# courtois-neuromod/phantom_vlb

Measured on AMD Instinct MI355X. Metric: clips/sec fine-tune VideoLLaMA2-7B+LoRA->2k-voxel head, 1/2/4/8 MI355X, higher is better.
Workload: dtype bf16; 1 GPU; configs[2]: VideoLLaMA2-7B + LoRA r=16 + 2k-voxel head, bf16; clips_per_gpu=3, global_batch=3, seq_len=2048, frames=12, num_target=2048, weights=random-init, comm=none

## Files before the change

### include/vlb.h

```cpp
#ifndef VLB_H
#define VLB_H

#include <stdint.h>

#ifdef __cplusplus
extern "C" {
#endif
#if defined(__GNUC__) || defined(__clang__)
#pragma GCC visibility push(default)
#endif

#define VLB_OK 0
#define VLB_ERR_INVALID (-1)
#define VLB_ERR_LAUNCH (-2)

#define VLB_ABI_VERSION 2

#define VLB_ACT_NONE 0
#define VLB_ACT_QUICK_GELU 1
#define VLB_ACT_GELU 2
#define VLB_ACT_SILU 3
#define VLB_ACT_SWIGLU_PAIR 4
#define VLB_ACT_SWIGLU_BWD 5

// ... 18 lines not shown
                              void* stream);

int vlb_gemm_bf16_masked_pair_ws(const void* A, int lda, const void* W, int ldw, void* C, int ldc, int M, int N, int K,
                                 const void* A2, int lda2, const void* W2, int ldw2, float drop_p, uint32_t seed,
                                 void* ws, int64_t ws_bytes, void* stream);

int vlb_gemm_masked_pair_swiglu_bwd(const void* dY, int lddy, const void* Wt, int ldw, const void* gu, int ldgu, void* dgu,
                                    int lddgu, int M, int ff, int K, const void* U, int ldu, const void* At, int ldat,
                                    float drop_p, uint32_t seed, void* ws, int64_t ws_bytes, void* stream);

int vlb_gemm_kernel_choice(int M, int N, int K, int K2);

int vlb_transpose_bf16(const void* in, void* out, int R, int C, void* stream);

int vlb_attention_fwd(const void* q, int ldq, const void* k, int ldk, const void* v, int ldv, void* out, int ldo,
                      float* lse, const uint8_t* key_mask, int B, int S, int Hq, int Hkv, int D, int causal,
                      float scale, const int* cu_rows, void* stream);

int vlb_attention_bwd(const void* q, int ldq, const void* k, int ldk, const void* v, int ldv, const void* out,
                      int ldo, const void* dout, int lddo, const float* lse, const uint8_t* key_mask, void* dq,
                      int lddq, void* dk, int lddk, void* dv, int lddv, float* delta, float* dq_acc, int B, int S,
                      int Hq, int Hkv, int D, int causal, float scale, const int* cu_rows, int total_rows,
                      void* stream);

int vlb_rmsnorm_fwd(const void* x, const void* w, void* y, int rows, int dim, float eps, void* stream);
int vlb_rmsnorm_bwd(const void* x, const void* w, const void* dy, const void* dx_in, void* dx, int rows, int dim,
                    float eps, void* stream);
int vlb_layernorm_fwd(const void* x, const void* w, const void* b, const void* residual, void* y, int rows, int dim,
                      float eps, int act, void* stream);

int vlb_rope_inplace(void* x, int ld, const float* cos_t, const float* sin_t, int rows, int S, int heads, int D,
                     int sign, const int* pos, void* stream);
int vlb_swiglu_fwd(const void* gu, void* out, int rows, int ff, void* stream);
int vlb_swiglu_bwd(const void* gu, const void* dout, void* dgu, int rows, int ff, void* stream);
int vlb_add_bf16(const void* a, const void* b, void* y, int64_t n, void* stream);

int vlb_patchify(const float* vision, void* patches, int N, int H, int W, int P, int Kpad, void* stream);
int vlb_vit_assemble(const void* patch_emb, const void* cls, const void* pos, void* tokens, int N, int G, int D,
                     void* stream);
int vlb_drop_cls(const void* tokens, void* out, int N, int G, int D, void* stream);

int vlb_dwconv3x3(const void* x, const void* w, void* y, int N, int H, int W, int C, void* stream);
int vlb_se_pool(const void* x, void* pooled, int N, int HW, int C, void* stream);
int vlb_se_scale(const void* x, const void* gate, void* y, int N, int HW, int C, void* stream);
int vlb_im2col3d_k2s2p1(const void* x, void* cols, int B, int T, int H, int W, int C, void* stream);

// ... 127 lines not shown
```

### phantom_vlb_amd/_lib.py

```python
from __future__ import annotations

import ctypes
import os
from ctypes import c_char_p, c_double, c_float, c_int, c_int64, c_void_p

import torch

_HERE = os.path.dirname(os.path.abspath(__file__))
LIB_PATH = os.environ.get("VLB_LIB") or os.path.join(_HERE, "libvlb.so")
IS_PRODUCT_LIB = os.path.abspath(LIB_PATH) == os.path.join(_HERE, "libvlb.so")

P, I, F, L = c_void_p, c_int, c_float, c_int64

SIGNATURES = {
    "vlb_abi_version": [],
    "vlb_last_error": [],
    "vlb_gemm_bf16": [P, I, P, I, P, I, I, I, I, P, P, I, I, P, I, P, I, I, P],
    "vlb_gemm_bf16_ws": [P, I, P, I, P, I, I, I, I, P, P, I, I, P, I, P, I, I, P, L, P],
    "vlb_gemm_swiglu_save": [P, I, P, I, P, I, P, I, I, I, I, P, I, P, I, I, P, L, P],
    "vlb_gemm_workspace_bytes": [],
    "vlb_gemm_plan": [I, I, I, I, I],
    "vlb_gemm_kernel_choice": [I, I, I, I],
    "vlb_transpose_bf16": [P, P, I, I, P],
    "vlb_attention_fwd": [P, I, P, I, P, I, P, I, P, P, I, I, I, I, I, I, F, P, P],
    "vlb_attention_bwd": [P, I, P, I, P, I, P, I, P, I, P, P, P, I, P, I, P, I, P, P, I, I, I, I, I, I, F, P, I, P],
    "vlb_rmsnorm_fwd": [P, P, P, I, I, F, P],
    "vlb_rmsnorm_bwd": [P, P, P, P, P, I, I, F, P],
    "vlb_layernorm_fwd": [P, P, P, P, P, I, I, F, I, P],
    "vlb_rope_inplace": [P, I, P, P, I, I, I, I, I, P, P],
    "vlb_swiglu_fwd": [P, P, I, I, P],
    "vlb_swiglu_bwd": [P, P, P, I, I, P],
    "vlb_add_bf16": [P, P, P, L, P],
    "vlb_patchify": [P, P, I, I, I, I, I, P],
    "vlb_vit_assemble": [P, P, P, P, I, I, I, P],
    "vlb_drop_cls": [P, P, I, I, I, P],
    "vlb_dwconv3x3": [P, P, P, I, I, I, I, P],
    "vlb_se_pool": [P, P, I, I, I, P],
    "vlb_se_scale": [P, P, P, I, I, I, P],
    "vlb_im2col3d_k2s2p1": [P, P, I, I, I, I, I, P],
    "vlb_splice_embed": [P, P, P, P, P, P, I, I, I, I, L, I, P, P, P],
    "vlb_weight_mask": [P, P, P, P, I, I, I, I, I, I, P],
    "vlb_head_partial_rows": [I],
    "vlb_head_ws_floats": [I, I, I, I],
    "vlb_head_fwd": [P] * 19 + [I, I, I, I, F, F, P, P],
    "vlb_head_bwd": [P] * 24 + [I, I, I, I, F, F, F, F, P, I, P],
    "vlb_feature_cache_store": [P] * 5 + [I, I, I, P],
    "vlb_head_fwd_cached": [P] * 19 + [I, I, I, I, F, F, P],
    "vlb_head_bwd_cached": [P] * 20 + [I, I, I, F, F, F, F, P],
# ... 97 lines not shown
```

### phantom_vlb_amd/backbone.py

```python
from __future__ import annotations

import math

import torch

from . import ops
from .geometry import Geometry, VIDEO_TOKEN_ID, decoder_linears

BF16 = torch.bfloat16
V_PRE = "model.vision_tower.vision_tower.vision_model"
M_PRE = "model.mm_projector"


def _bf(t, dev):
    return t.detach().to(device=dev, dtype=BF16).contiguous()


class Weights:

    def __init__(self, g: Geometry, sd: dict, device, keep_transposed: bool = False, gate_up_interleaved: bool | None = None):
        self.g = g
        self.dev = device
        d = device
        w = sd[f"{V_PRE}.embeddings.patch_embedding.weight"].reshape(g.vit_dim, -1)
# ... 188 lines not shown

    def connector(self, feats, B):
        g, w = self.g, self.w
        x = feats
        for blk in w.s1:
            x = self._bottleneck(x, blk, B * g.num_frames, g.grid)
        cols = ops.im2col3d(x, B, g.num_frames, g.grid, g.grid, g.dim)
        x = ops.gemm(cols, w.sampler_w, bias=w.sampler_b, act=ops.ACT_SILU)
        for blk in w.s2:
            x = self._bottleneck(x, blk, B * g.ds_frames, g.ds_grid)
        x = ops.gemm(x, w.ro0[0], bias=w.ro0[1], act=ops.ACT_GELU)
        return ops.gemm(x, w.ro2[0], bias=w.ro2[1])

    def attention(self, qkv, key_mask, B, layout=None, need_lse=False):
        g, w = self.g, self.w
        qd, kd = g.q_dim, g.kv_dim
        ops.rope_(qkv, w.rope_cos, w.rope_sin, B, g.max_len, g.heads + g.kv_heads, g.head_dim,
                  pos=None if layout is None else layout.pos)
        return ops.attention_fwd(qkv[:, :qd], qkv[:, qd:qd + kd], qkv[:, qd + kd:], B, g.max_len, g.heads, g.kv_heads,
                                 g.head_dim, True, g.head_dim ** -0.5, key_mask=key_mask, need_lse=need_lse, layout=layout)

    def attention_bwd(self, qkv, a, d_a, lse, key_mask, B, layout, delta):
        g, w = self.g, self.w
        dqkv = ops.attention_bwd(qkv, g.q_dim, g.kv_dim, a, d_a, lse, key_mask, B, g.max_len, g.heads, g.kv_heads,
                                 g.head_dim, True, g.head_dim ** -0.5, layout=layout, delta=delta)
        ops.rope_(dqkv, w.rope_cos, w.rope_sin, B, g.max_len, g.heads + g.kv_heads, g.head_dim, sign=-1,
                  pos=None if layout is None else layout.pos)
        return dqkv

    def decoder_layer(self, x, lw, key_mask, B, S, save=None, layout=None):
        g = self.g
        assert S == g.max_len, "the decoder runs at the geometry's sequence length (rope tables, attention)"
        h = ops.rmsnorm(x, lw["in_norm"], g.rms_eps)
        qkv = ops.gemm(h, lw["wqkv"])
        a = self.attention(qkv, key_mask, B, layout)
        x = ops.gemm(a, lw["wo"], residual=x)
        h = ops.rmsnorm(x, lw["post_norm"], g.rms_eps)
        if lw.get("wgu_il") is not None:
            h = ops.gemm(h, lw["wgu_il"], act=ops.ACT_SWIGLU_PAIR)
        else:
            h = ops.swiglu(ops.gemm(h, lw["wgu"]))
        return ops.gemm(h, lw["wdown"], residual=x)

    def named_modules(self):
        from .litmodule import _LinearInfo
        g = self.g
        for i in range(g.vit_layers):
            p = f"{V_PRE}.encoder.layers.{i}"
            for n in ("q_proj", "k_proj", "v_proj", "out_proj"):
                yield f"{p}.self_attn.{n}", _LinearInfo(g.vit_dim, g.vit_dim)
            yield f"{p}.mlp.fc1", _LinearInfo(g.vit_ff, g.vit_dim)
# ... 148 lines not shown
```

### phantom_vlb_amd/csrc/attention.hip

```cpp
#include "common.hpp"

namespace {

constexpr int KV = 64;
constexpr int QW = 32;
constexpr int NW = 4;
constexpr int QB = QW * NW;
constexpr float NEG = -1e30f;

__device__ __forceinline__ void glds16(const void* g, void* l) {
  __builtin_amdgcn_global_load_lds((const void __attribute__((address_space(1)))*)g,
                                   (void __attribute__((address_space(3)))*)l, 16, 0, 0);
}

typedef short s16x4 __attribute__((ext_vector_type(4)));

__device__ __forceinline__ s16x4 tr_read_asm(const char* lds_ptr) {
  s16x4 v;
  const unsigned a = (unsigned)(uintptr_t)(const char __attribute__((address_space(3)))*)lds_ptr;
  asm volatile("ds_read_b64_tr_b16 %0, %1" : "=v"(v) : "v"(a));
  return v;
}
__device__ __forceinline__ void lds_wait_all() {
  asm volatile("s_waitcnt lgkmcnt(0)" ::: "memory");
// ... 458 lines not shown

__global__ __launch_bounds__(256) void attn_dkdv_reduce_kernel(const bf16* __restrict__ part, bf16* __restrict__ dk, int lddk,
                                                               bf16* __restrict__ dv, int lddv, int Hq, int Hkv, int64_t total) {
  const int64_t i = blockIdx.x * (int64_t)blockDim.x + threadIdx.x;
  if (i >= total) return;
  const int c = i & 15, which = (i >> 4) & 1;
  const int hkv = (int)((i >> 5) % Hkv);
  const int64_t row = (i >> 5) / Hkv;
  const int gsz = Hq / Hkv;
  float acc[8] = {0.f, 0.f, 0.f, 0.f, 0.f, 0.f, 0.f, 0.f};
  const bf16* src = part + (row * Hq + (int64_t)hkv * gsz) * 256 + which * 128 + c * 8;
  for (int j = 0; j < gsz; ++j) {
    const bf16x8 v = *reinterpret_cast<const bf16x8*>(src + (int64_t)j * 256);
#pragma unroll
    for (int e = 0; e < 8; ++e) acc[e] += (float)v[e];
  }
  bf16x8 o;
#pragma unroll
  for (int e = 0; e < 8; ++e) o[e] = (bf16)acc[e];
  bf16* dst = which ? dv + row * lddv : dk + row * lddk;
  *reinterpret_cast<bf16x8*>(dst + hkv * 128 + c * 8) = o;
}

struct AttnDqArgs {
  const bf16* q; const bf16* k; const bf16* v; const bf16* dout;
  const float* lse; const float* delta; const uint8_t* mask; const int* cu;
  bf16* dq;
  int ldq, ldk, ldv, lddo, lddq;
  int B, S, Hq, Hkv;
  float scale;
};

template <bool CAUSAL>
__global__ __launch_bounds__(256, 2) void attn_bwd_dq_kernel(AttnDqArgs p) {
  constexpr int D = 128, ROWB = 256, TILE = KV * ROWB, KS = 8, DT = 4;
  extern __shared__ __attribute__((aligned(16))) char smem[];

  const int tid = threadIdx.x, lane = tid & 63;
  const int wave = __builtin_amdgcn_readfirstlane(tid >> 6);
  const int nqb = (p.S + QB - 1) / QB;
  const int per_qb = p.Hq * p.B, slot = blockIdx.x / per_qb;
  const int qb = CAUSAL ? (nqb - 1 - slot) : slot;
  const int hq = xcd_head((blockIdx.x % per_qb) % p.Hq, p.Hq), b = (blockIdx.x % per_qb) / p.Hq;
  const int hkv = hq / (p.Hq / p.Hkv);
  const int Sb = p.cu ? p.cu[b + 1] - p.cu[b] : p.S;
  const int64_t row0 = p.cu ? p.cu[b] : (int64_t)b * p.S;
  if (qb * QB >= Sb) return;
  const int q0 = qb * QB + wave * QW;
  const int ql = lane & 31, h = lane >> 5;
  const int qrow = q0 + ql;
  const int qr = min(qrow, Sb - 1);

  bf16x8 qf[KS], dof[KS];
  {
    const bf16* qp = p.q + (row0 + qr) * p.ldq + hq * D + 8 * h;
    const bf16* dp = p.dout + (row0 + qr) * p.lddo + hq * D + 8 * h;
#pragma unroll
    for (int ks = 0; ks < KS; ++ks) {
      qf[ks] = *reinterpret_cast<const bf16x8*>(qp + 16 * ks);
      dof[ks] = *reinterpret_cast<const bf16x8*>(dp + 16 * ks);
    }
  }
  const float lse_q = p.lse[((int64_t)b * p.Hq + hq) * p.S + qr];
  const float delta_q = p.delta[((int64_t)b * p.Hq + hq) * p.S + qr];
  const float c2 = p.scale * 1.44269504088896341f;
  const float lse2 = (lse_q > -1e37f) ? lse_q * 1.44269504088896341f : 1e37f;

  f32x16 dqt[DT];
#pragma unroll
  for (int i = 0; i < DT; ++i)
#pragma unroll
    for (int r = 0; r < 16; ++r) dqt[i][r] = 0.f;

  const int q_hi = min(qb * QB + QB, Sb) - 1;
  const int ntiles = CAUSAL ? (q_hi / KV + 1) : (Sb + KV - 1) / KV;
  const bf16* kbase = p.k + row0 * p.ldk + hkv * D;
  const bf16* vbase = p.v + row0 * p.ldv + hkv * D;

  const int sr = lane >> 4, sp = lane & 15;
  auto stage = [&](int buf, int t) {
    char* kb = smem + buf * 2 * TILE; char* vb = kb + TILE;
#pragma unroll
    for (int i = 0; i < 4; ++i) {
      const int r = (4 * i + wave) * 4 + sr;
      const int key = min(t * KV + r, Sb - 1);
      glds16(kbase + (int64_t)key * p.ldk + (sp ^ sw2(r)) * 8, kb + (4 * i + wave) * 1024);
      glds16(vbase + (int64_t)key * p.ldv + (sp ^ sw2(r)) * 8, vb + (4 * i + wave) * 1024);
    }
  };
  stage(0, 0);
  asm volatile("s_waitcnt vmcnt(0)" ::: "memory");
  __syncthreads();

  const int g1 = (lane >> 4) & 1, li = lane & 15, tq = li >> 2, tp = li & 3;
  int row_rd[KS];
#pragma unroll
  for (int ks = 0; ks < KS; ++ks) row_rd[ks] = ql * ROWB + (((2 * ks + h) ^ sw2(ql)) << 4);
  int tr_rd[DT][2];
#pragma unroll
  for (int dt = 0; dt < DT; ++dt)
#pragma unroll
    for (int e = 0; e < 2; ++e) {
      const int r = 4 * h + tq + 8 * e;
      tr_rd[dt][e] = r * ROWB + (((4 * dt + 2 * g1 + (tp >> 1)) ^ sw2(r)) << 4) + (tp & 1) * 8;
    }

  for (int t = 0; t < ntiles; ++t) {
    const int cur = t & 1;
    if (t + 1 < ntiles) stage(cur ^ 1, t + 1);
    const char* kb = smem + cur * 2 * TILE; const char* vb = kb + TILE;
    const int key0 = t * KV;
    const bool active = !CAUSAL || (key0 <= q0 + QW - 1);
    if (active) {
// ... 47 lines not shown
      for (int s = 0; s < 2; ++s)
#pragma unroll
        for (int s2 = 0; s2 < 2; ++s2) {
          bf16x8 df;
#pragma unroll
          for (int j = 0; j < 8; ++j) df[j] = (bf16)st[s][8 * s2 + j];
          const int roff = (32 * s + 16 * s2) * ROWB;
#pragma unroll
          for (int dt = 0; dt < DT; ++dt) {
            const s16x4 lo = __builtin_amdgcn_ds_read_tr16_b64_v4i16(
                (s16x4 __attribute__((address_space(3)))*)(kb + tr_rd[dt][0] + roff));
            const s16x4 hi = __builtin_amdgcn_ds_read_tr16_b64_v4i16(
                (s16x4 __attribute__((address_space(3)))*)(kb + tr_rd[dt][1] + roff));
            dqt[dt] = __builtin_amdgcn_mfma_f32_32x32x16_bf16(join8(lo, hi), df, dqt[dt], 0, 0, 0);
          }
        }
    }
    asm volatile("s_waitcnt vmcnt(0)" ::: "memory");
    __syncthreads();
  }

  if (qrow < Sb) {
    bf16* op = p.dq + (row0 + qrow) * p.lddq + hq * D;
#pragma unroll
    for (int dt = 0; dt < DT; ++dt)
#pragma unroll
      for (int g = 0; g < 4; ++g) {
        bf16x4 o;
#pragma unroll
        for (int e = 0; e < 4; ++e) o[e] = (bf16)dqt[dt][4 * g + e];
        *reinterpret_cast<bf16x4*>(op + 32 * dt + 8 * g + 4 * h) = o;
      }
  }
}

}

extern "C" int vlb_attention_bwd(const void* q, int ldq, const void* k, int ldk, const void* v, int ldv, const void* out,
                                 int ldo, const void* dout, int lddo, const float* lse, const uint8_t* key_mask, void* dq,
                                 int lddq, void* dk, int lddk, void* dv, int lddv, float* delta, float* dq_acc, int B,
                                 int S, int Hq, int Hkv, int D, int causal, float scale, const int* cu_rows, int total_rows,
                                 void* stream) {
  VLB_REQUIRE(q && k && v && out && dout && lse && dq && dk && dv && delta, "attention_bwd: null operand");
  VLB_REQUIRE(dq_acc || Hq == Hkv, "attention_bwd: the [rows, Hq, D] fp32-sized workspace is required");
  VLB_REQUIRE(D == 128, "attention_bwd: head dim %d unsupported (only 128: the decoder)", D);
  VLB_REQUIRE(B > 0 && S > 0 && Hq > 0 && Hkv > 0 && Hq % Hkv == 0, "attention_bwd: bad shape");
  VLB_REQUIRE(ldq % 8 == 0 && ldk % 8 == 0 && ldv % 8 == 0 && ldo % 8 == 0 && lddo % 8 == 0 && lddq % 8 == 0 &&
                  lddk % 4 == 0 && lddv % 4 == 0, "attention_bwd: strides must keep vector alignment");
  VLB_REQUIRE(((((uintptr_t)q | (uintptr_t)k | (uintptr_t)v | (uintptr_t)out | (uintptr_t)dout) % 16) == 0) &&
                  ((uintptr_t)dq % 8 == 0), "attention_bwd: misaligned pointer");
  hipStream_t st = as_stream(stream);
  const int64_t rows = cu_rows ? (int64_t)total_rows : (int64_t)B * S;
  VLB_REQUIRE(rows > 0 && rows <= (int64_t)B * S, "attention_bwd: total_rows=%d out of range", total_rows);
  const int64_t th = rows * Hq;
  hipLaunchKernelGGL(attn_delta_kernel, dim3((unsigned)((th + 15) / 16)), dim3(256), 0, st, (const bf16*)out, ldo,
                     (const bf16*)dout, lddo, delta, S, Hq, B, cu_rows, th);
  VLB_LAUNCH_CHECK();
  AttnBwdArgs a{(const bf16*)q, (const bf16*)k, (const bf16*)v, (const bf16*)dout, lse, delta, key_mask, cu_rows,
                (bf16*)dk, (bf16*)dv, dq_acc, ldq, ldk, ldv, lddo, lddk, lddv, B, S, Hq, Hkv, scale, g_attn_ablate};
  dim3 grid((S + BK_KEYS - 1) / BK_KEYS, Hkv, B);
  {
    const int gsz = Hq / Hkv;
    VLB_REQUIRE(gsz == 1 || dq_acc, "attention_bwd: the workspace (fp32 [rows, Hq, D]) is required for grouped-query heads");
    VLB_REQUIRE(lddk % 8 == 0 && lddv % 8 == 0 && (((uintptr_t)dk | (uintptr_t)dv) % 16) == 0, "attention_bwd: dk/dv rows must be 16-byte aligned");
    constexpr int LDS_KV = BK_KEYS * 256 + 4 * BQ * 256 + 512;
    static const hipError_t k1 = hipFuncSetAttribute(reinterpret_cast<const void*>(&attn_bwd_dkdv_kernel<true>), hipFuncAttributeMaxDynamicSharedMemorySize, LDS_KV);
    static const hipError_t k2 = hipFuncSetAttribute(reinterpret_cast<const void*>(&attn_bwd_dkdv_kernel<false>), hipFuncAttributeMaxDynamicSharedMemorySize, LDS_KV);
    if (k1 != hipSuccess || k2 != hipSuccess) { vlb_set_error("attention_bwd: LDS reservation failed (dk/dv)"); return VLB_ERR_LAUNCH; }
    bf16* part = reinterpret_cast<bf16*>(dq_acc);
    dim3 gridh(grid.x * Hq * B);
    if (causal) hipLaunchKernelGGL(attn_bwd_dkdv_kernel<true>, gridh, dim3(256), LDS_KV, st, a, part);
    else hipLaunchKernelGGL(attn_bwd_dkdv_kernel<false>, gridh, dim3(256), LDS_KV, st, a, part);
    VLB_LAUNCH_CHECK();
    if (gsz > 1) {
      const int64_t tot = rows * Hkv * 32;
      hipLaunchKernelGGL(attn_dkdv_reduce_kernel, dim3((unsigned)((tot + 255) / 256)), dim3(256), 0, st, part, (bf16*)dk, lddk,
                         (bf16*)dv, lddv, Hq, Hkv, tot);
      VLB_LAUNCH_CHECK();
    }
  }
  AttnDqArgs d{(const bf16*)q, (const bf16*)k, (const bf16*)v, (const bf16*)dout, lse, delta, key_mask, cu_rows,
               (bf16*)dq, ldq, ldk, ldv, lddo, lddq, B, S, Hq, Hkv, scale};
  constexpr int LDS_DQ = 2 * 2 * KV * 256;
  static const hipError_t q1 = hipFuncSetAttribute(reinterpret_cast<const void*>(&attn_bwd_dq_kernel<true>), hipFuncAttributeMaxDynamicSharedMemorySize, LDS_DQ);
  static const hipError_t q2 = hipFuncSetAttribute(reinterpret_cast<const void*>(&attn_bwd_dq_kernel<false>), hipFuncAttributeMaxDynamicSharedMemorySize, LDS_DQ);
  if (q1 != hipSuccess || q2 != hipSuccess) { vlb_set_error("attention_bwd: LDS reservation failed (dq)"); return VLB_ERR_LAUNCH; }
  dim3 gq(((S + QB - 1) / QB) * Hq * B);
  if (causal) hipLaunchKernelGGL(attn_bwd_dq_kernel<true>, gq, dim3(256), LDS_DQ, st, d);
  else hipLaunchKernelGGL(attn_bwd_dq_kernel<false>, gq, dim3(256), LDS_DQ, st, d);
  VLB_LAUNCH_CHECK();
  return VLB_OK;
}

#ifdef VLB_TOOLS
extern "C" void vlb_attn_set_ablation(int bits) { g_attn_ablate = bits & 3; }
#endif
```

### phantom_vlb_amd/csrc/common.hpp

```cpp
#pragma once
#include <hip/hip_runtime.h>
#include <stdint.h>
#include <stdio.h>
#include <string.h>

#include "../../include/vlb.h"

typedef __bf16 bf16;
typedef __bf16 bf16x2 __attribute__((ext_vector_type(2)));
typedef __bf16 bf16x4 __attribute__((ext_vector_type(4)));
typedef __bf16 bf16x8 __attribute__((ext_vector_type(8)));
typedef float f32x2 __attribute__((ext_vector_type(2)));
typedef float f32x4 __attribute__((ext_vector_type(4)));
typedef float f32x16 __attribute__((ext_vector_type(16)));
typedef unsigned int u32x2 __attribute__((ext_vector_type(2)));
typedef unsigned int u32x4 __attribute__((ext_vector_type(4)));

#define VLB_WAVE 64

void vlb_set_error(const char* fmt, ...);

#define VLB_REQUIRE(cond, ...)                 \
  do {                                         \
    if (!(cond)) {                             \
// ... 22 lines not shown

__device__ __forceinline__ float wave_sum(float v) {
#pragma unroll
  for (int o = 32; o > 0; o >>= 1) v += __shfl_xor(v, o, 64);
  return v;
}
__device__ __forceinline__ float wave_max(float v) {
#pragma unroll
  for (int o = 32; o > 0; o >>= 1) v = fmaxf(v, __shfl_xor(v, o, 64));
  return v;
}

__device__ __forceinline__ float block_sum(float v, float* red) {
  v = wave_sum(v);
  const int w = threadIdx.x >> 6, nw = blockDim.x >> 6;
  __syncthreads();
  if ((threadIdx.x & 63) == 0) red[w] = v;
  __syncthreads();
  float t = 0.f;
  for (int i = 0; i < nw; ++i) t += red[i];
  return t;
}

__device__ __forceinline__ float sigmoid_f(float x) { return __builtin_amdgcn_rcpf(1.f + __expf(-x)); }
__device__ __forceinline__ float silu_f(float x) { return x * sigmoid_f(x); }
__device__ __forceinline__ float quick_gelu_f(float x) { return x * sigmoid_f(1.702f * x); }
__device__ __forceinline__ float gelu_erf_f(float x) { return 0.5f * x * (1.f + erff(x * 0.70710678118654752f)); }

__device__ __forceinline__ int mx_shared_exp(float amax) {
  int E = -127;
  if (amax > 0.f) {
    int e; const float f = frexpf(amax / 448.f, &e);
    E = (f == 0.5f) ? e - 1 : e;
    E = max(-127, min(127, E));
  }
  return E;
}
__device__ __forceinline__ uint32_t mx_pack4(float a, float b, float c, float d, float inv) {
  int pk = 0;
  pk = __builtin_amdgcn_cvt_pk_fp8_f32(a * inv, b * inv, pk, false);
  pk = __builtin_amdgcn_cvt_pk_fp8_f32(c * inv, d * inv, pk, true);
  return (uint32_t)pk;
}
__device__ __forceinline__ void mx_quantize_lane8(const float (&v)[8], uint8_t* qrow, uint8_t* srow, int c, int lane) {
  float amax = 0.f;
#pragma unroll
// ... 28 lines not shown
```

### phantom_vlb_amd/csrc/ops.hip

```cpp
#include "common.hpp"

namespace {

constexpr int kMaxBlocks = 256 * 8;

__device__ __forceinline__ void load8(const bf16* p, float (&v)[8]) {
  const bf16x8 t = *reinterpret_cast<const bf16x8*>(p);
#pragma unroll
  for (int i = 0; i < 8; ++i) v[i] = (float)t[i];
}
__device__ __forceinline__ void store8(bf16* p, const float (&v)[8]) {
  bf16x8 t;
#pragma unroll
  for (int i = 0; i < 8; ++i) t[i] = (bf16)v[i];
  *reinterpret_cast<bf16x8*>(p) = t;
}

__global__ __launch_bounds__(256) void rmsnorm_fwd_kernel(const bf16* __restrict__ x, const bf16* __restrict__ w,
                                                          bf16* __restrict__ y, int rows, int dim, float eps) {
  const int row = blockIdx.x * 4 + (threadIdx.x >> 6), lane = threadIdx.x & 63;
  if (row >= rows) return;
  const bf16* xr = x + (int64_t)row * dim;
  float ss = 0.f;
  for (int c = lane * 8; c < dim; c += 512) {
// ... 235 lines not shown
    }
    if (act != VLB_ACT_NONE) {
#pragma unroll
      for (int i = 0; i < 8; ++i) v[i] = act_f(v[i], act);
    }
    store8(yr + c, v);
  }
}

__global__ void rope_kernel(bf16* __restrict__ x, int ld, const float* __restrict__ cs, const float* __restrict__ sn,
                            int S, int heads, int D, float sign, const int* __restrict__ pos, int64_t total) {
  const int half = D >> 1, cpr = half >> 3;
  for (int64_t idx = blockIdx.x * (int64_t)blockDim.x + threadIdx.x; idx < total; idx += (int64_t)gridDim.x * blockDim.x) {
    const int ch = idx % cpr;
    const int h = (idx / cpr) % heads;
    const int64_t tok = idx / ((int64_t)cpr * heads);
    const int s = pos ? pos[tok] : (int)(tok % S);
    bf16* p = x + tok * ld + h * D + ch * 8;
    float a[8], b[8]; load8(p, a); load8(p + half, b);
    const float* c = cs + (int64_t)s * half + ch * 8;
    const float* n = sn + (int64_t)s * half + ch * 8;
    float oa[8], ob[8];
#pragma unroll
    for (int i = 0; i < 8; ++i) {
      const float co = c[i], si = sign * n[i];
      oa[i] = a[i] * co - b[i] * si;
      ob[i] = b[i] * co + a[i] * si;
    }
    store8(p, oa); store8(p + half, ob);
  }
}

__global__ void swiglu_fwd_kernel(const bf16* __restrict__ gu, bf16* __restrict__ out, int ff, int64_t total) {
  const int cpr = ff >> 3;
  for (int64_t idx = blockIdx.x * (int64_t)blockDim.x + threadIdx.x; idx < total; idx += (int64_t)gridDim.x * blockDim.x) {
    const int64_t r = idx / cpr; const int c = (idx % cpr) * 8;
    float g[8], u[8]; load8(gu + r * 2 * ff + c, g); load8(gu + r * 2 * ff + ff + c, u);
#pragma unroll
    for (int i = 0; i < 8; ++i) g[i] = silu_f(g[i]) * u[i];
    store8(out + r * ff + c, g);
  }
}
__global__ void swiglu_fwd_q8_kernel(const bf16* __restrict__ gu, bf16* __restrict__ out, uint8_t* __restrict__ q, int ldq,
                                     uint8_t* __restrict__ s, int lds_, int ff, int64_t total) {
  const int cpr = ff >> 3;
  for (int64_t idx = blockIdx.x * (int64_t)blockDim.x + threadIdx.x; idx < total; idx += (int64_t)gridDim.x * blockDim.x) {
    const int64_t r = idx / cpr; const int c = (idx % cpr) * 8;
    float g[8], u[8]; load8(gu + r * 2 * ff + c, g); load8(gu + r * 2 * ff + ff + c, u);
#pragma unroll
    for (int i = 0; i < 8; ++i) g[i] = (float)(bf16)(silu_f(g[i]) * u[i]);
    store8(out + r * ff + c, g);
// ... 593 lines not shown
```

### phantom_vlb_amd/ops.py

```python
from __future__ import annotations

import torch

from ._lib import check, lib

ACT_NONE, ACT_QUICK_GELU, ACT_GELU, ACT_SILU, ACT_SWIGLU_PAIR = 0, 1, 2, 3, 4
BF16 = torch.bfloat16


def _stream():
    return torch.cuda.current_stream().cuda_stream


def _p(t):
    return None if t is None else t.data_ptr()


def _dev(t):
    if not t.is_cuda:
        raise RuntimeError("phantom_vlb_amd ops need GPU tensors (no CPU fallback)")
    return t


class _GemmProbe:
# ... 229 lines not shown
    if layout is not None and layout.packed:
        B, S, cu, rows = layout.B, layout.smax, layout.cu, layout.rows
    assert q.shape[0] == rows, f"attention_fwd: {q.shape[0]} rows, layout has {rows}"
    if out is None:
        out = torch.empty(rows, Hq * D, dtype=BF16, device=q.device)
    lse = torch.empty(B, Hq, S, dtype=torch.float32, device=q.device) if need_lse else None
    check(lib.vlb_attention_fwd(q.data_ptr(), q.stride(0), k.data_ptr(), k.stride(0), v.data_ptr(), v.stride(0),
                                out.data_ptr(), out.stride(0), _p(lse), _p(key_mask), B, S, Hq, Hkv, D,
                                1 if causal else 0, float(scale), _p(cu), _stream()), "vlb_attention_fwd")
    return (out, lse) if need_lse else out


_ATTN_WS = [None]


def _attn_workspace(n_floats, device):
    ws = _ATTN_WS[0]
    if ws is None or ws.numel() < n_floats or ws.device != device:
        ws = _ATTN_WS[0] = torch.empty(n_floats, dtype=torch.float32, device=device)
    return ws


def attention_bwd(qkv, qd, kd, out, dout, lse, key_mask, B, S, Hq, Hkv, D, causal, scale, layout=None, delta=None,
                  dq_acc=None):
    cu, rows = None, B * S
    if layout is not None and layout.packed:
        B, S, cu, rows = layout.B, layout.smax, layout.cu, layout.rows
    assert qkv.shape[0] == rows and dout.shape[0] == rows
    if delta is None:
        delta = torch.empty(B, Hq, S, dtype=torch.float32, device=qkv.device)
    if dq_acc is None and Hq != Hkv:
        dq_acc = _attn_workspace(rows * qd, qkv.device)
    assert delta.numel() >= B * Hq * S and (dq_acc is None or dq_acc.numel() >= rows * qd)
    dqkv = torch.empty_like(qkv)
    check(lib.vlb_attention_bwd(qkv.data_ptr(), qkv.stride(0), qkv[:, qd:].data_ptr(), qkv.stride(0),
                                qkv[:, qd + kd:].data_ptr(), qkv.stride(0), out.data_ptr(), out.stride(0),
                                dout.data_ptr(), dout.stride(0), lse.data_ptr(), _p(key_mask),
                                dqkv.data_ptr(), dqkv.stride(0), dqkv[:, qd:].data_ptr(), dqkv.stride(0),
                                dqkv[:, qd + kd:].data_ptr(), dqkv.stride(0), delta.data_ptr(), _p(dq_acc),
                                B, S, Hq, Hkv, D, 1 if causal else 0, float(scale), _p(cu), rows, _stream()),
          "vlb_attention_bwd")
    return dqkv


def rmsnorm(x, w, eps, out=None):
    rows, dim = x.shape
    if out is None:
        out = torch.empty_like(x)
    check(lib.vlb_rmsnorm_fwd(_dev(x).data_ptr(), w.data_ptr(), out.data_ptr(), rows, dim, eps, _stream()), "vlb_rmsnorm_fwd")
    return out


def rmsnorm_bwd(x, w, dy, eps, dx_in=None, out=None):
    rows, dim = x.shape
    if out is None:
        out = torch.empty_like(x)
    check(lib.vlb_rmsnorm_bwd(_dev(x).data_ptr(), w.data_ptr(), dy.data_ptr(), _p(dx_in), out.data_ptr(), rows, dim, eps,
                              _stream()), "vlb_rmsnorm_bwd")
    return out


def layernorm(x, w, b, eps, residual=None, act=ACT_NONE, out=None):
    rows, dim = x.shape
    if out is None:
# ... 291 lines not shown
```

Baseline: 15.18 clips/s.

## Fuse delta computation and inverse RoPE into attention backward kernels

```diff
diff --git a/include/vlb.h b/include/vlb.h
--- a/include/vlb.h
+++ b/include/vlb.h
@@ -64,6 +64,11 @@
                       int lddq, void* dk, int lddk, void* dv, int lddv, float* delta, float* dq_acc, int B, int S,
                       int Hq, int Hkv, int D, int causal, float scale, const int* cu_rows, int total_rows,
                       void* stream);
+int vlb_attention_bwd_rope(const void* q, int ldq, const void* k, int ldk, const void* v, int ldv, const void* out,
+                           int ldo, const void* dout, int lddo, const float* lse, const uint8_t* key_mask, void* dq,
+                           int lddq, void* dk, int lddk, void* dv, int lddv, float* delta, float* dq_acc, int B, int S,
+                           int Hq, int Hkv, int D, int causal, float scale, const int* cu_rows, int total_rows,
+                           const float* cos_t, const float* sin_t, const int* pos, void* stream);
 
 int vlb_rmsnorm_fwd(const void* x, const void* w, void* y, int rows, int dim, float eps, void* stream);
 int vlb_rmsnorm_bwd(const void* x, const void* w, const void* dy, const void* dx_in, void* dx, int rows, int dim,
diff --git a/phantom_vlb_amd/_lib.py b/phantom_vlb_amd/_lib.py
--- a/phantom_vlb_amd/_lib.py
+++ b/phantom_vlb_amd/_lib.py
@@ -24,6 +24,8 @@
     "vlb_transpose_bf16": [P, P, I, I, P],
     "vlb_attention_fwd": [P, I, P, I, P, I, P, I, P, P, I, I, I, I, I, I, F, P, P],
     "vlb_attention_bwd": [P, I, P, I, P, I, P, I, P, I, P, P, P, I, P, I, P, I, P, P, I, I, I, I, I, I, F, P, I, P],
+    "vlb_attention_bwd_rope": [P, I, P, I, P, I, P, I, P, I, P, P, P, I, P, I, P, I, P, P, I, I, I, I, I, I, F, P, I, P, P, P,
+                               P],
     "vlb_rmsnorm_fwd": [P, P, P, I, I, F, P],
     "vlb_rmsnorm_bwd": [P, P, P, P, P, I, I, F, P],
     "vlb_layernorm_fwd": [P, P, P, P, P, I, I, F, I, P],
diff --git a/phantom_vlb_amd/backbone.py b/phantom_vlb_amd/backbone.py
--- a/phantom_vlb_amd/backbone.py
+++ b/phantom_vlb_amd/backbone.py
@@ -234,11 +234,9 @@
 
     def attention_bwd(self, qkv, a, d_a, lse, key_mask, B, layout, delta):
         g, w = self.g, self.w
-        dqkv = ops.attention_bwd(qkv, g.q_dim, g.kv_dim, a, d_a, lse, key_mask, B, g.max_len, g.heads, g.kv_heads,
-                                 g.head_dim, True, g.head_dim ** -0.5, layout=layout, delta=delta)
-        ops.rope_(dqkv, w.rope_cos, w.rope_sin, B, g.max_len, g.heads + g.kv_heads, g.head_dim, sign=-1,
-                  pos=None if layout is None else layout.pos)
-        return dqkv
+        return ops.attention_bwd(qkv, g.q_dim, g.kv_dim, a, d_a, lse, key_mask, B, g.max_len, g.heads, g.kv_heads,
+                                 g.head_dim, True, g.head_dim ** -0.5, layout=layout, delta=delta,
+                                 rope=(w.rope_cos, w.rope_sin, None if layout is None else layout.pos))
 
     def decoder_layer(self, x, lw, key_mask, B, S, save=None, layout=None):
         g = self.g
diff --git a/phantom_vlb_amd/csrc/attention.hip b/phantom_vlb_amd/csrc/attention.hip
--- a/phantom_vlb_amd/csrc/attention.hip
+++ b/phantom_vlb_amd/csrc/attention.hip
@@ -504,6 +504,48 @@
   *reinterpret_cast<bf16x8*>(dst + hkv * 128 + c * 8) = o;
 }
 
+__global__ __launch_bounds__(256) void attn_dkdv_reduce_rope_kernel(const bf16* __restrict__ part, bf16* __restrict__ dk, int lddk,
+                                                                    bf16* __restrict__ dv, int lddv, int Hq, int Hkv,
+                                                                    const float* __restrict__ cs, const float* __restrict__ sn,
+                                                                    const int* __restrict__ pos, int S, int64_t total) {
+  const int64_t i = blockIdx.x * (int64_t)blockDim.x + threadIdx.x;
+  if (i >= total) return;
+  const int j = i & 15, which = j >> 3;
+  const int hkv = (int)((i >> 4) % Hkv);
+  const int64_t row = (i >> 4) / Hkv;
+  const int gsz = Hq / Hkv;
+  const int c0 = which ? 2 * (j - 8) : j, c1 = which ? c0 + 1 : j + 8;
+  float a0[8], a1[8];
+#pragma unroll
+  for (int e = 0; e < 8; ++e) { a0[e] = 0.f; a1[e] = 0.f; }
+  const bf16* src = part + (row * Hq + (int64_t)hkv * gsz) * 256 + which * 128;
+  for (int g = 0; g < gsz; ++g) {
+    const bf16x8 v0 = *reinterpret_cast<const bf16x8*>(src + (int64_t)g * 256 + c0 * 8);
+    const bf16x8 v1 = *reinterpret_cast<const bf16x8*>(src + (int64_t)g * 256 + c1 * 8);
+#pragma unroll
+    for (int e = 0; e < 8; ++e) { a0[e] += (float)v0[e]; a1[e] += (float)v1[e]; }
+  }
+  bf16x8 o0, o1;
+#pragma unroll
+  for (int e = 0; e < 8; ++e) { o0[e] = (bf16)a0[e]; o1[e] = (bf16)a1[e]; }
+  if (!which) {
+    const int s = pos ? pos[row] : (int)(row % S);
+    const float* c = cs + (int64_t)s * 64 + c0 * 8;
+    const float* n = sn + (int64_t)s * 64 + c0 * 8;
+    const f32x4 cl = *reinterpret_cast<const f32x4*>(c), ch = *reinterpret_cast<const f32x4*>(c + 4);
+    const f32x4 nl = *reinterpret_cast<const f32x4*>(n), nh = *reinterpret_cast<const f32x4*>(n + 4);
+#pragma unroll
+    for (int e = 0; e < 8; ++e) {
+      float ra, rb;
+      rope_rotate((float)o0[e], (float)o1[e], e < 4 ? cl[e & 3] : ch[e & 3], -(e < 4 ? nl[e & 3] : nh[e & 3]), ra, rb);
+      o0[e] = (bf16)ra; o1[e] = (bf16)rb;
+    }
+  }
+  bf16* dst = (which ? dv + row * lddv : dk + row * lddk) + hkv * 128;
+  *reinterpret_cast<bf16x8*>(dst + c0 * 8) = o0;
+  *reinterpret_cast<bf16x8*>(dst + c1 * 8) = o1;
+}
+
 struct AttnDqArgs {
   const bf16* q; const bf16* k; const bf16* v; const bf16* dout;
   const float* lse; const float* delta; const uint8_t* mask; const int* cu;
@@ -511,9 +553,11 @@
   int ldq, ldk, ldv, lddo, lddq;
   int B, S, Hq, Hkv;
   float scale;
+  const bf16* out; float* delta_w; const float* cs; const float* sn; const int* pos;
+  int ldo;
 };
 
-template <bool CAUSAL>
+template <bool CAUSAL, bool FUSED>
 __global__ __launch_bounds__(256, 2) void attn_bwd_dq_kernel(AttnDqArgs p) {
   constexpr int D = 128, ROWB = 256, TILE = KV * ROWB, KS = 8, DT = 4;
   extern __shared__ __attribute__((aligned(16))) char smem[];
@@ -544,7 +588,17 @@
     }
   }
   const float lse_q = p.lse[((int64_t)b * p.Hq + hq) * p.S + qr];
-  const float delta_q = p.delta[((int64_t)b * p.Hq + hq) * p.S + qr];
+  float delta_q = 0.f;
+  bf16x8 of[FUSED ? KS : 1];
+  int pos_q = 0;
+  if constexpr (FUSED) {
+    const bf16* op = p.out + (row0 + qr) * p.ldo + hq * D + 8 * h;
+#pragma unroll
+    for (int ks = 0; ks < KS; ++ks) of[ks] = *reinterpret_cast<const bf16x8*>(op + 16 * ks);
+    pos_q = *(p.pos ? p.pos + (row0 + qr) : reinterpret_cast<const int*>(p.lse));
+  } else {
+    delta_q = p.delta[((int64_t)b * p.Hq + hq) * p.S + qr];
+  }
   const float c2 = p.scale * 1.44269504088896341f;
   const float lse2 = (lse_q > -1e37f) ? lse_q * 1.44269504088896341f : 1e37f;
 
@@ -571,6 +625,31 @@
     }
   };
   stage(0, 0);
+  if constexpr (FUSED) {
+    __builtin_amdgcn_sched_barrier(0);
+    float part[KS], oth[KS];
+    {
+#pragma clang fp contract(off)
+#pragma unroll
+      for (int ks = 0; ks < KS; ++ks) {
+        float s = 0.f;
+#pragma unroll
+        for (int i = 0; i < 8; ++i) s = s + (float)of[ks][i] * (float)dof[ks][i];
+        part[ks] = s;
+      }
+    }
+#pragma unroll
+    for (int ks = 0; ks < KS; ++ks) oth[ks] = __shfl_xor(part[ks], 32, 64);
+    float t[16];
+#pragma unroll
+    for (int ks = 0; ks < KS; ++ks) { t[2 * ks] = h ? oth[ks] : part[ks]; t[2 * ks + 1] = h ? part[ks] : oth[ks]; }
+#pragma unroll
+    for (int w = 8; w > 0; w >>= 1)
+#pragma unroll
+      for (int c = 0; c < w; ++c) t[c] = t[c] + t[c + w];
+    delta_q = t[0];
+    if (qrow < Sb && h == 0) p.delta_w[((int64_t)b * p.Hq + hq) * p.S + qrow] = delta_q;
+  }
   asm volatile("s_waitcnt vmcnt(0)" ::: "memory");
   __syncthreads();
 
@@ -664,25 +743,54 @@
 
   if (qrow < Sb) {
     bf16* op = p.dq + (row0 + qrow) * p.lddq + hq * D;
-#pragma unroll
-    for (int dt = 0; dt < DT; ++dt)
-#pragma unroll
-      for (int g = 0; g < 4; ++g) {
-        bf16x4 o;
-#pragma unroll
-        for (int e = 0; e < 4; ++e) o[e] = (bf16)dqt[dt][4 * g + e];
-        *reinterpret_cast<bf16x4*>(op + 32 * dt + 8 * g + 4 * h) = o;
-      }
-  }
-}
-
-}
-
-extern "C" int vlb_attention_bwd(const void* q, int ldq, const void* k, int ldk, const void* v, int ldv, const void* out,
-                                 int ldo, const void* dout, int lddo, const float* lse, const uint8_t* key_mask, void* dq,
-                                 int lddq, void* dk, int lddk, void* dv, int lddv, float* delta, float* dq_acc, int B,
-                                 int S, int Hq, int Hkv, int D, int causal, float scale, const int* cu_rows, int total_rows,
-                                 void* stream) {
+    if constexpr (FUSED) {
+      const int spos = p.pos ? pos_q : p.cu ? (int)((unsigned)(row0 + qrow) % (unsigned)p.S) : qrow;
+      const float* cp = p.cs + (int64_t)spos * (D / 2) + 4 * h;
+      const float* np = p.sn + (int64_t)spos * (D / 2) + 4 * h;
+      f32x4 co[DT / 2][4], si[DT / 2][4];
+#pragma unroll
+      for (int dt = 0; dt < DT / 2; ++dt)
+#pragma unroll
+        for (int g = 0; g < 4; ++g) {
+          co[dt][g] = *reinterpret_cast<const f32x4*>(cp + 32 * dt + 8 * g);
+          si[dt][g] = *reinterpret_cast<const f32x4*>(np + 32 * dt + 8 * g);
+        }
+#pragma unroll
+      for (int dt = 0; dt < DT / 2; ++dt)
+#pragma unroll
+        for (int g = 0; g < 4; ++g) {
+          bf16x4 oa, ob;
+#pragma unroll
+          for (int e = 0; e < 4; ++e) {
+            float ra, rb;
+            rope_rotate((float)(bf16)dqt[dt][4 * g + e], (float)(bf16)dqt[dt + 2][4 * g + e], co[dt][g][e], -si[dt][g][e], ra, rb);
+            oa[e] = (bf16)ra; ob[e] = (bf16)rb;
+          }
+          *reinterpret_cast<bf16x4*>(op + 32 * dt + 8 * g + 4 * h) = oa;
+          *reinterpret_cast<bf16x4*>(op + 32 * (dt + 2) + 8 * g + 4 * h) = ob;
+        }
+    } else {
+#pragma unroll
+      for (int dt = 0; dt < DT; ++dt)
+#pragma unroll
+        for (int g = 0; g < 4; ++g) {
+          bf16x4 o;
+#pragma unroll
+          for (int e = 0; e < 4; ++e) o[e] = (bf16)dqt[dt][4 * g + e];
+          *reinterpret_cast<bf16x4*>(op + 32 * dt + 8 * g + 4 * h) = o;
+        }
+    }
+  }
+}
+
+}
+
+static int attention_bwd_impl(const void* q, int ldq, const void* k, int ldk, const void* v, int ldv, const void* out,
+                              int ldo, const void* dout, int lddo, const float* lse, const uint8_t* key_mask, void* dq,
+                              int lddq, void* dk, int lddk, void* dv, int lddv, float* delta, float* dq_acc, int B,
+                              int S, int Hq, int Hkv, int D, int causal, float scale, const int* cu_rows, int total_rows,
+                              const float* cos_t, const float* sin_t, const int* pos, void* stream) {
+  const bool fused = cos_t != nullptr;
   VLB_REQUIRE(q && k && v && out && dout && lse && dq && dk && dv && delta, "attention_bwd: null operand");
   VLB_REQUIRE(dq_acc || Hq == Hkv, "attention_bwd: the [rows, Hq, D] fp32-sized workspace is required");
   VLB_REQUIRE(D == 128, "attention_bwd: head dim %d unsupported (only 128: the decoder)", D);
@@ -691,20 +799,47 @@
                   lddk % 4 == 0 && lddv % 4 == 0, "attention_bwd: strides must keep vector alignment");
   VLB_REQUIRE(((((uintptr_t)q | (uintptr_t)k | (uintptr_t)v | (uintptr_t)out | (uintptr_t)dout) % 16) == 0) &&
                   ((uintptr_t)dq % 8 == 0), "attention_bwd: misaligned pointer");
+  VLB_REQUIRE(!fused || (sin_t && (((uintptr_t)cos_t | (uintptr_t)sin_t) % 16) == 0), "attention_bwd_rope: cos/sin tables must be 16-byte aligned");
   hipStream_t st = as_stream(stream);
   const int64_t rows = cu_rows ? (int64_t)total_rows : (int64_t)B * S;
   VLB_REQUIRE(rows > 0 && rows <= (int64_t)B * S, "attention_bwd: total_rows=%d out of range", total_rows);
-  const int64_t th = rows * Hq;
-  hipLaunchKernelGGL(attn_delta_kernel, dim3((unsigned)((th + 15) / 16)), dim3(256), 0, st, (const bf16*)out, ldo,
-                     (const bf16*)dout, lddo, delta, S, Hq, B, cu_rows, th);
-  VLB_LAUNCH_CHECK();
+  const int gsz = Hq / Hkv;
+  VLB_REQUIRE(gsz == 1 || dq_acc, "attention_bwd: the workspace (fp32 [rows, Hq, D]) is required for grouped-query heads");
+  VLB_REQUIRE(lddk % 8 == 0 && lddv % 8 == 0 && (((uintptr_t)dk | (uintptr_t)dv) % 16) == 0, "attention_bwd: dk/dv rows must be 16-byte aligned");
+
+  auto launch_dq = [&]() -> int {
+    AttnDqArgs d{(const bf16*)q, (const bf16*)k, (const bf16*)v, (const bf16*)dout, lse, delta, key_mask, cu_rows,
+                 (bf16*)dq, ldq, ldk, ldv, lddo, lddq, B, S, Hq, Hkv, scale, (const bf16*)out, delta, cos_t, sin_t, pos, ldo};
+    constexpr int LDS_DQ = 2 * 2 * KV * 256;
+    static const hipError_t q1 = hipFuncSetAttribute(reinterpret_cast<const void*>(&attn_bwd_dq_kernel<true, false>), hipFuncAttributeMaxDynamicSharedMemorySize, LDS_DQ);
+    static const hipError_t q2 = hipFuncSetAttribute(reinterpret_cast<const void*>(&attn_bwd_dq_kernel<false, false>), hipFuncAttributeMaxDynamicSharedMemorySize, LDS_DQ);
+    static const hipError_t q3 = hipFuncSetAttribute(reinterpret_cast<const void*>(&attn_bwd_dq_kernel<true, true>), hipFuncAttributeMaxDynamicSharedMemorySize, LDS_DQ);
+    static const hipError_t q4 = hipFuncSetAttribute(reinterpret_cast<const void*>(&attn_bwd_dq_kernel<false, true>), hipFuncAttributeMaxDynamicSharedMemorySize, LDS_DQ);
+    if (q1 != hipSuccess || q2 != hipSuccess || q3 != hipSuccess || q4 != hipSuccess) { vlb_set_error("attention_bwd: LDS reservation failed (dq)"); return VLB_ERR_LAUNCH; }
+    dim3 gq(((S + QB - 1) / QB) * Hq * B);
+    if (fused) {
+      if (causal) hipLaunchKernelGGL((attn_bwd_dq_kernel<true, true>), gq, dim3(256), LDS_DQ, st, d);
+      else hipLaunchKernelGGL((attn_bwd_dq_kernel<false, true>), gq, dim3(256), LDS_DQ, st, d);
+    } else {
+      if (causal) hipLaunchKernelGGL((attn_bwd_dq_kernel<true, false>), gq, dim3(256), LDS_DQ, st, d);
+      else hipLaunchKernelGGL((attn_bwd_dq_kernel<false, false>), gq, dim3(256), LDS_DQ, st, d);
+    }
+    VLB_LAUNCH_CHECK();
+    return VLB_OK;
+  };
+
+  if (fused) {
+    if (const int rc = launch_dq()) return rc;
+  } else {
+    const int64_t th = rows * Hq;
+    hipLaunchKernelGGL(attn_delta_kernel, dim3((unsigned)((th + 15) / 16)), dim3(256), 0, st, (const bf16*)out, ldo,
+                       (const bf16*)dout, lddo, delta, S, Hq, B, cu_rows, th);
+    VLB_LAUNCH_CHECK();
+  }
   AttnBwdArgs a{(const bf16*)q, (const bf16*)k, (const bf16*)v, (const bf16*)dout, lse, delta, key_mask, cu_rows,
                 (bf16*)dk, (bf16*)dv, dq_acc, ldq, ldk, ldv, lddo, lddk, lddv, B, S, Hq, Hkv, scale, g_attn_ablate};
   dim3 grid((S + BK_KEYS - 1) / BK_KEYS, Hkv, B);
   {
-    const int gsz = Hq / Hkv;
-    VLB_REQUIRE(gsz == 1 || dq_acc, "attention_bwd: the workspace (fp32 [rows, Hq, D]) is required for grouped-query heads");
-    VLB_REQUIRE(lddk % 8 == 0 && lddv % 8 == 0 && (((uintptr_t)dk | (uintptr_t)dv) % 16) == 0, "attention_bwd: dk/dv rows must be 16-byte aligned");
     constexpr int LDS_KV = BK_KEYS * 256 + 4 * BQ * 256 + 512;
     static const hipError_t k1 = hipFuncSetAttribute(reinterpret_cast<const void*>(&attn_bwd_dkdv_kernel<true>), hipFuncAttributeMaxDynamicSharedMemorySize, LDS_KV);
     static const hipError_t k2 = hipFuncSetAttribute(reinterpret_cast<const void*>(&attn_bwd_dkdv_kernel<false>), hipFuncAttributeMaxDynamicSharedMemorySize, LDS_KV);
@@ -714,24 +849,41 @@
     if (causal) hipLaunchKernelGGL(attn_bwd_dkdv_kernel<true>, gridh, dim3(256), LDS_KV, st, a, part);
     else hipLaunchKernelGGL(attn_bwd_dkdv_kernel<false>, gridh, dim3(256), LDS_KV, st, a, part);
     VLB_LAUNCH_CHECK();
-    if (gsz > 1) {
+    if (gsz > 1 && fused) {
+      const int64_t tot = rows * Hkv * 16;
+      hipLaunchKernelGGL(attn_dkdv_reduce_rope_kernel, dim3((unsigned)((tot + 255) / 256)), dim3(256), 0, st, part, (bf16*)dk,
+                         lddk, (bf16*)dv, lddv, Hq, Hkv, cos_t, sin_t, pos, S, tot);
+      VLB_LAUNCH_CHECK();
+    } else if (gsz > 1) {
       const int64_t tot = rows * Hkv * 32;
       hipLaunchKernelGGL(attn_dkdv_reduce_kernel, dim3((unsigned)((tot + 255) / 256)), dim3(256), 0, st, part, (bf16*)dk, lddk,
                          (bf16*)dv, lddv, Hq, Hkv, tot);
       VLB_LAUNCH_CHECK();
-    }
-  }
-  AttnDqArgs d{(const bf16*)q, (const bf16*)k, (const bf16*)v, (const bf16*)dout, lse, delta, key_mask, cu_rows,
-               (bf16*)dq, ldq, ldk, ldv, lddo, lddq, B, S, Hq, Hkv, scale};
-  constexpr int LDS_DQ = 2 * 2 * KV * 256;
-  static const hipError_t q1 = hipFuncSetAttribute(reinterpret_cast<const void*>(&attn_bwd_dq_kernel<true>), hipFuncAttributeMaxDynamicSharedMemorySize, LDS_DQ);
-  static const hipError_t q2 = hipFuncSetAttribute(reinterpret_cast<const void*>(&attn_bwd_dq_kernel<false>), hipFuncAttributeMaxDynamicSharedMemorySize, LDS_DQ);
-  if (q1 != hipSuccess || q2 != hipSuccess) { vlb_set_error("attention_bwd: LDS reservation failed (dq)"); return VLB_ERR_LAUNCH; }
-  dim3 gq(((S + QB - 1) / QB) * Hq * B);
-  if (causal) hipLaunchKernelGGL(attn_bwd_dq_kernel<true>, gq, dim3(256), LDS_DQ, st, d);
-  else hipLaunchKernelGGL(attn_bwd_dq_kernel<false>, gq, dim3(256), LDS_DQ, st, d);
-  VLB_LAUNCH_CHECK();
-  return VLB_OK;
+    } else if (fused) {
+      if (const int rc = vlb_rope_inplace(dk, lddk, cos_t, sin_t, (int)rows, S, Hkv, D, -1, pos, stream)) return rc;
+    }
+  }
+  return fused ? VLB_OK : launch_dq();
+}
+
+extern "C" int vlb_attention_bwd(const void* q, int ldq, const void* k, int ldk, const void* v, int ldv, const void* out,
+                                 int ldo, const void* dout, int lddo, const float* lse, const uint8_t* key_mask, void* dq,
+                                 int lddq, void* dk, int lddk, void* dv, int lddv, float* delta, float* dq_acc, int B,
+                                 int S, int Hq, int Hkv, int D, int causal, float scale, const int* cu_rows, int total_rows,
+                                 void* stream) {
+  return attention_bwd_impl(q, ldq, k, ldk, v, ldv, out, ldo, dout, lddo, lse, key_mask, dq, lddq, dk, lddk, dv, lddv, delta,
+                            dq_acc, B, S, Hq, Hkv, D, causal, scale, cu_rows, total_rows, nullptr, nullptr, nullptr, stream);
+}
+
+extern "C" int vlb_attention_bwd_rope(const void* q, int ldq, const void* k, int ldk, const void* v, int ldv, const void* out,
+                                      int ldo, const void* dout, int lddo, const float* lse, const uint8_t* key_mask,
+                                      void* dq, int lddq, void* dk, int lddk, void* dv, int lddv, float* delta,
+                                      float* dq_acc, int B, int S, int Hq, int Hkv, int D, int causal, float scale,
+                                      const int* cu_rows, int total_rows, const float* cos_t, const float* sin_t,
+                                      const int* pos, void* stream) {
+  VLB_REQUIRE(cos_t && sin_t, "attention_bwd_rope: null cos/sin table");
+  return attention_bwd_impl(q, ldq, k, ldk, v, ldv, out, ldo, dout, lddo, lse, key_mask, dq, lddq, dk, lddk, dv, lddv, delta,
+                            dq_acc, B, S, Hq, Hkv, D, causal, scale, cu_rows, total_rows, cos_t, sin_t, pos, stream);
 }
 
 #ifdef VLB_TOOLS
diff --git a/phantom_vlb_amd/csrc/common.hpp b/phantom_vlb_amd/csrc/common.hpp
--- a/phantom_vlb_amd/csrc/common.hpp
+++ b/phantom_vlb_amd/csrc/common.hpp
@@ -68,6 +68,13 @@
   return t;
 }
 
+__device__ __forceinline__ void rope_rotate(float a, float b, float co, float si, float& oa, float& ob) {
+#pragma clang fp contract(off)
+  const float bs = b * si, as = a * si;
+  oa = __builtin_fmaf(a, co, -bs);
+  ob = __builtin_fmaf(b, co, as);
+}
+
 __device__ __forceinline__ float sigmoid_f(float x) { return __builtin_amdgcn_rcpf(1.f + __expf(-x)); }
 __device__ __forceinline__ float silu_f(float x) { return x * sigmoid_f(x); }
 __device__ __forceinline__ float quick_gelu_f(float x) { return x * sigmoid_f(1.702f * x); }
diff --git a/phantom_vlb_amd/csrc/ops.hip b/phantom_vlb_amd/csrc/ops.hip
--- a/phantom_vlb_amd/csrc/ops.hip
+++ b/phantom_vlb_amd/csrc/ops.hip
@@ -281,11 +281,7 @@
     const float* n = sn + (int64_t)s * half + ch * 8;
     float oa[8], ob[8];
 #pragma unroll
-    for (int i = 0; i < 8; ++i) {
-      const float co = c[i], si = sign * n[i];
-      oa[i] = a[i] * co - b[i] * si;
-      ob[i] = b[i] * co + a[i] * si;
-    }
+    for (int i = 0; i < 8; ++i) rope_rotate(a[i], b[i], c[i], sign * n[i], oa[i], ob[i]);
     store8(p, oa); store8(p + half, ob);
   }
 }
diff --git a/phantom_vlb_amd/ops.py b/phantom_vlb_amd/ops.py
--- a/phantom_vlb_amd/ops.py
+++ b/phantom_vlb_amd/ops.py
@@ -275,7 +275,7 @@
 
 
 def attention_bwd(qkv, qd, kd, out, dout, lse, key_mask, B, S, Hq, Hkv, D, causal, scale, layout=None, delta=None,
-                  dq_acc=None):
+                  dq_acc=None, rope=None):
     cu, rows = None, B * S
     if layout is not None and layout.packed:
         B, S, cu, rows = layout.B, layout.smax, layout.cu, layout.rows
@@ -286,13 +286,19 @@
         dq_acc = _attn_workspace(rows * qd, qkv.device)
     assert delta.numel() >= B * Hq * S and (dq_acc is None or dq_acc.numel() >= rows * qd)
     dqkv = torch.empty_like(qkv)
-    check(lib.vlb_attention_bwd(qkv.data_ptr(), qkv.stride(0), qkv[:, qd:].data_ptr(), qkv.stride(0),
-                                qkv[:, qd + kd:].data_ptr(), qkv.stride(0), out.data_ptr(), out.stride(0),
-                                dout.data_ptr(), dout.stride(0), lse.data_ptr(), _p(key_mask),
-                                dqkv.data_ptr(), dqkv.stride(0), dqkv[:, qd:].data_ptr(), dqkv.stride(0),
-                                dqkv[:, qd + kd:].data_ptr(), dqkv.stride(0), delta.data_ptr(), _p(dq_acc),
-                                B, S, Hq, Hkv, D, 1 if causal else 0, float(scale), _p(cu), rows, _stream()),
-          "vlb_attention_bwd")
+    args = (qkv.data_ptr(), qkv.stride(0), qkv[:, qd:].data_ptr(), qkv.stride(0),
+            qkv[:, qd + kd:].data_ptr(), qkv.stride(0), out.data_ptr(), out.stride(0),
+            dout.data_ptr(), dout.stride(0), lse.data_ptr(), _p(key_mask),
+            dqkv.data_ptr(), dqkv.stride(0), dqkv[:, qd:].data_ptr(), dqkv.stride(0),
+            dqkv[:, qd + kd:].data_ptr(), dqkv.stride(0), delta.data_ptr(), _p(dq_acc),
+            B, S, Hq, Hkv, D, 1 if causal else 0, float(scale), _p(cu), rows)
+    if rope is None:
+        check(lib.vlb_attention_bwd(*args, _stream()), "vlb_attention_bwd")
+    else:
+        cos, sin, pos = rope
+        assert cos.dtype == sin.dtype == torch.float32 and cos.shape[1] == sin.shape[1] == D // 2
+        assert pos is None or pos.shape[0] == rows
+        check(lib.vlb_attention_bwd_rope(*args, cos.data_ptr(), sin.data_ptr(), _p(pos), _stream()), "vlb_attention_bwd_rope")
     return dqkv
 
 
```

Result: no change. 15.17 clips/s (-0.0%).
